# RolandFaure/Hairsplitter

Measured on AMD Instinct MI355X. Metric: aligned read-bp/sec through call_variants+separate_reads, higher is better.
Workload: dtype u8

## Files before the change

### hairsplitter_amd/csrc/hs_kernels_graph.hip

```cpp
#pragma once

namespace hsdev {

static __device__ __forceinline__ float wave_max_f01(float v) { return __int_as_float(wave_max_i32(__float_as_int(v))); }

template <int FILTER>
static __device__ __forceinline__ void next_level(const float* __restrict__ dv, int m, int lane, float cur, float below, float above,
                                                  int extra_zeros, float* v_out, int* c_out) {
    float best = -1.f;
    for (int j = lane; j < m; j += 64) {
        const float d = dv[j];
        const bool ok = FILTER == 0 ? (d != 1.f) : (d > below && d != 1.f && d < above);
        if (ok && d < cur && d > best) best = d;
    }
    if (FILTER == 0 && extra_zeros > 0 && 0.f < cur && best < 0.f) best = 0.f;
    const int key = best < 0.f ? -1 : __float_as_int(best);
    const int kmax = wave_max_i32(key);
    const float vv = kmax < 0 ? -1.f : __int_as_float(kmax);
    int c = 0;
    if (kmax >= 0) {
        for (int j = lane; j < m; j += 64) {
            const float d = dv[j];
            const bool ok = FILTER == 0 ? (d != 1.f) : (d > below && d != 1.f && d < above);
            if (ok && d == vv) c++;
        }
        c = wave_sum_i32(c);
        if (FILTER == 0 && vv == 0.f) c += extra_zeros;
    }
    *v_out = vv; *c_out = c;
}

template <bool LM>
__global__ __launch_bounds__(256) void k_read_graph_rows(
    const int32_t* __restrict__ sim, const int32_t* __restrict__ diff, const int64_t* __restrict__ ctg_out_off,
    const int32_t* __restrict__ ctg_n, const int32_t* __restrict__ win_contig, const int64_t* __restrict__ win_mask_off,
    const int32_t* __restrict__ mask_ids, const int32_t* __restrict__ row_win, const int64_t* __restrict__ win_bits_off,
    int row_base, int n_rows, float below, int cap, unsigned long long* __restrict__ bits, unsigned long long* __restrict__ amb_head ,
    int32_t* __restrict__ amb_rows, int amb_cap, const int64_t* __restrict__ win_mat_off, int es ,
    long long* __restrict__ amb_stage_off , int32_t* __restrict__ stage_sim, int32_t* __restrict__ stage_diff,
    long long stage_cap, const int32_t* __restrict__ pos_rank , const int64_t* __restrict__ rank_off) {
    extern __shared__ unsigned char s_dyn[];
    const int lane = lane_id();
    const int wv = wave_id(), waves = (int)(blockDim.x >> 6);
    const int row = row_base + (int)blockIdx.x * waves + wv;
    if (row >= row_base + n_rows) return;
    float* __restrict__ dv = reinterpret_cast<float*>(s_dyn) + (size_t)wv * 2 * cap;
    int* __restrict__ tv = reinterpret_cast<int*>(dv + cap);
    const int w = row_win[row];
    const int64_t m0 = win_mask_off[w];
    const int m = (int)(win_mask_off[w + 1] - m0);
    const int i = row - (int)m0;
    const int c = win_contig[w];
    const int N = ctg_n[c];
    const int32_t* __restrict__ ids = mask_ids + m0;
    const int r1 = ids[i];
    const int32_t* __restrict__ prk = (!LM && pos_rank) ? pos_rank + rank_off[c] : nullptr;
    const int r1k = prk ? prk[r1] : r1;
    const int32_t* __restrict__ srow = LM ? sim + (win_mat_off[w] + (int64_t)i * m) * es : sim + (ctg_out_off[c] + (int64_t)r1k * N) * es;
    const int32_t* __restrict__ drow = LM ? diff + (win_mat_off[w] + (int64_t)i * m) * es : diff + (ctg_out_off[c] + (int64_t)r1k * N) * es;
    auto give_up = [&]() {
        const int len = LM ? m : N;
        long long so = -1;
        if (lane == 0) {
            const long long k = (long long)atomicAdd(&amb_head[0], 1ull);
            if (k < amb_cap) {
                amb_rows[k] = row;
                if (stage_sim) { so = (long long)atomicAdd(&amb_head[1], (unsigned long long)len); if (so + len > stage_cap) so = -1; }
                amb_stage_off[k] = so;
            }
        }
        so = (long long)(((unsigned long long)(unsigned)__builtin_amdgcn_readlane((int)(so & 0xffffffffll), 0)) |
                         ((unsigned long long)(unsigned)__builtin_amdgcn_readlane((int)((unsigned long long)so >> 32), 0) << 32));
        if (so >= 0) for (int j = lane; j < len; j += 64) { const int64_t at = (int64_t)(prk ? prk[j] : j) * es; stage_sim[so + j] = srow[at]; stage_diff[so + j] = drow[at]; }
    };
    if (m > cap || N < 2 || !(below >= 0.f)) { give_up(); return; }

    int max_compat = 0;
    bool nan_l = false;
    for (int j = lane; j < m; j += 64) {
        const int r = ids[j];
        const int64_t at = (int64_t)(LM ? j : (prk ? prk[r] : r)) * es;
        const int s = srow[at], dd = drow[at];
        float d = 0.f;
        if (LM) {
            if (r != r1) {
                const float df = (float)(dd - 1 > 0 ? dd - 1 : 0);
                d = 1.f - df / (float)(s + dd);
                if (s > max_compat) max_compat = s;
            }
        } else if (r != r1 && s > 0) {
            const float df = (float)(dd - 1 > 0 ? dd - 1 : 0);
            d = 1.f - df / (float)(s + dd);
            if (s > max_compat) max_compat = s;
        }
        dv[j] = d; tv[j] = r != r1 ? s + dd : 0x7fffffff;
    }
    max_compat = wave_max_i32(max_compat);
    const double thr = 0.7 * (double)max_compat;
    for (int j = lane; j < m; j += 64) {
        if ((double)tv[j] < thr) dv[j] = 0.f;
        if (LM && dv[j] != dv[j]) nan_l = true;
    }
    wave_lds_sync();
    if (LM && __ballot(nan_l) != 0ull) { give_up(); return; }

    const int extra_zeros = N - m;
    float s0, s1; int c0, ones = 0;
    {
        float best = 0.f;
        for (int j = lane; j < m; j += 64) { const float d = dv[j]; if (d > best) best = d; if (d == 1.f) ones++; }
        s0 = wave_max_f01(best);
        ones = wave_sum_i32(ones);
        int cnt = 0; float second = -1.f;
        for (int j = lane; j < m; j += 64) { const float d = dv[j]; if (d == s0) cnt++; else if (d > second) second = d; }
        c0 = wave_sum_i32(cnt) + (s0 == 0.f ? extra_zeros : 0);
        if (extra_zeros > 0 && s0 > 0.f && second < 0.f) second = 0.f;
        const int key = second < 0.f ? -1 : __float_as_int(second);
        const int kmax = wave_max_i32(key);
        s1 = c0 >= 2 ? s0 : (kmax < 0 ? -1.f : __int_as_float(kmax));
    }
    float above = s0 - (s0 - s1) * 3;
    if (above == 1.f && ones < N) {
        const int idx = (ones + 4) < (N - 1) ? (ones + 4) : (N - 1);
        int k = idx - ones;
        float cur = 2.f, v = 0.f; int cc = 0;
        for (int it = 0; it < 5; ++it) {
            next_level<0>(dv, m, lane, cur, below, above, extra_zeros, &v, &cc);
            if (cc == 0) { v = 0.f; break; }
            if (k < cc) break;
            k -= cc; cur = v;
        }
        above = v;
    }
    const int mw64 = (m + 63) >> 6;
    unsigned long long* __restrict__ wb = bits + win_bits_off[w];
    int nA = 0;
    for (int j = lane; j < m; j += 64) { const float d = dv[j]; if (d > below && (d == 1.f || d >= above)) nA++; }
    nA = wave_sum_i32(nA);
    float cut = 3.f;
    if (nA < 5) {
        const int need = 5 - nA;
        int nB = 0;
        for (int j = lane; j < m; j += 64) { const float d = dv[j]; if (d > below && d != 1.f && d < above) nB++; }
        nB = wave_sum_i32(nB);
        if (nB > 0 && nB <= need) cut = -1.f;
        else if (nB > need) {
            int remaining = need; float cur = 2.f, v = 0.f; int cc = 0;
            bool ambiguous = false;
            for (int it = 0; it < 5; ++it) {
                next_level<1>(dv, m, lane, cur, below, above, 0, &v, &cc);
                if (remaining <= cc) { ambiguous = remaining != cc; break; }
                remaining -= cc; cur = v;
            }
            if (ambiguous) { give_up(); return; }
            cut = v;
        }
    }
    for (int j = lane; j < m; j += 64) {
        const float d = dv[j];
        const bool take = d > below && ((d == 1.f || d >= above) || (d != 1.f && d < above && d >= cut));
        if (take) {
            atomicOr(&wb[(int64_t)i * mw64 + (j >> 6)], 1ull << (j & 63));
            atomicOr(&wb[(int64_t)j * mw64 + (i >> 6)], 1ull << (i & 63));
        }
    }
}

__global__ __launch_bounds__(256) void k_read_graph_fetch_rows(
    const int32_t* __restrict__ sim, const int32_t* __restrict__ diff, const int64_t* __restrict__ src_off,
    const int32_t* __restrict__ len, const int64_t* __restrict__ dst_off, int32_t* __restrict__ out_sim, int32_t* __restrict__ out_diff, int es) {
    const int k = (int)blockIdx.x;
    const int n = len[k];
    for (int j = (int)threadIdx.x; j < n; j += 256) { out_sim[dst_off[k] + j] = sim[(src_off[k] + j) * es]; out_diff[dst_off[k] + j] = diff[(src_off[k] + j) * es]; }
}

__global__ __launch_bounds__(256) void k_read_graph_patch(const int64_t* __restrict__ base, const int32_t* __restrict__ mw64,
                                                         const int32_t* __restrict__ pi, const int32_t* __restrict__ pj, int n,
                                                         unsigned long long* __restrict__ bits) {
    const int k = (int)(blockIdx.x * 256 + threadIdx.x);
    if (k >= n) return;
    unsigned long long* wb = bits + base[k];
    atomicOr(&wb[(int64_t)pi[k] * mw64[k] + (pj[k] >> 6)], 1ull << (pj[k] & 63));
    atomicOr(&wb[(int64_t)pj[k] * mw64[k] + (pi[k] >> 6)], 1ull << (pi[k] & 63));
}

__global__ __launch_bounds__(256) void k_read_graph_degrees(const unsigned long long* __restrict__ bits, const int32_t* __restrict__ row_win,
                                                           const int64_t* __restrict__ win_mask_off, const int64_t* __restrict__ win_bits_off,
                                                           int n_rows, int32_t* __restrict__ deg) {
    const int row = (int)(blockIdx.x * 256 + threadIdx.x);
    if (row >= n_rows) return;
    const int w = row_win[row];
    const int m = (int)(win_mask_off[w + 1] - win_mask_off[w]);
    const int mw64 = (m + 63) >> 6;
    const unsigned long long* p = bits + win_bits_off[w] + (int64_t)(row - win_mask_off[w]) * mw64;
    int d = 0;
    for (int k = 0; k < mw64; ++k) d += __popcll(p[k]);
    deg[row] = d;
}

#define HS_SCAN_TILE 4096
__global__ __launch_bounds__(256) void k_scan_tile_sums(const int32_t* __restrict__ in, int n, long long* __restrict__ tile_sum) {
    __shared__ int s_w[4];
    const int t = (int)threadIdx.x;
    const int64_t base = (int64_t)blockIdx.x * HS_SCAN_TILE;
    int s = 0;
#pragma unroll
    for (int k = 0; k < HS_SCAN_TILE / 256; ++k) { const int64_t i = base + k * 256 + t; if (i < n) s += in[i]; }
    s = wave_sum_i32(s);
    if ((t & 63) == 0) s_w[t >> 6] = s;
    __syncthreads();
    if (t == 0) tile_sum[blockIdx.x] = (long long)s_w[0] + s_w[1] + s_w[2] + s_w[3];
}

__global__ __launch_bounds__(1024) void k_scan_tile_offsets(const long long* __restrict__ tile_sum, int n_tiles, long long* __restrict__ tile_off,
                                                           int64_t* __restrict__ total_out) {
    __shared__ long long s_part[1024];
    const int t = (int)threadIdx.x;
    long long carry = 0;
    for (int base = 0; base < n_tiles; base += 1024) {
        const long long v = base + t < n_tiles ? tile_sum[base + t] : 0;
        s_part[t] = v;
        __syncthreads();
        for (int d = 1; d < 1024; d <<= 1) {
            const long long a = t >= d ? s_part[t - d] : 0;
            __syncthreads();
            s_part[t] += a;
            __syncthreads();
        }
        if (base + t < n_tiles) tile_off[base + t] = carry + s_part[t] - v;
        carry += s_part[1023];
        __syncthreads();
    }
    if (t == 0) *total_out = carry;
}

__global__ __launch_bounds__(256) void k_scan_apply(const int32_t* __restrict__ in, int n, const long long* __restrict__ tile_off,
                                                    int64_t* __restrict__ out) {
    __shared__ int s_w[2][4];
    const int t = (int)threadIdx.x, lane = t & 63, wv = t >> 6;
    const int64_t base = (int64_t)blockIdx.x * HS_SCAN_TILE;
    long long run = tile_off[blockIdx.x];
#pragma unroll 1
    for (int k = 0; k < HS_SCAN_TILE / 256; ++k) {
        const int64_t i = base + k * 256 + t;
        const int v = i < n ? in[i] : 0;
        const int incl = wave_scan_incl(v);
        if (lane == 63) s_w[k & 1][wv] = incl;
        __syncthreads();
        const int w0 = s_w[k & 1][0], w1 = s_w[k & 1][1], w2 = s_w[k & 1][2], w3 = s_w[k & 1][3];
        const int before = (wv > 0 ? w0 : 0) + (wv > 1 ? w1 : 0) + (wv > 2 ? w2 : 0);
        if (i < n) out[i] = run + before + incl - v;
        run += (long long)w0 + w1 + w2 + w3;
    }
}

__global__ __launch_bounds__(256) void k_read_graph_fill(const unsigned long long* __restrict__ bits, const int32_t* __restrict__ row_win,
                                                        const int64_t* __restrict__ win_mask_off, const int64_t* __restrict__ win_bits_off,
                                                        const int64_t* __restrict__ nbr_off, int n_rows, int32_t* __restrict__ nbr) {
    const int row = (int)(blockIdx.x * 256 + threadIdx.x);
    if (row >= n_rows) return;
    const int w = row_win[row];
    const int64_t m0 = win_mask_off[w];
    const int m = (int)(win_mask_off[w + 1] - m0);
    const int mw64 = (m + 63) >> 6;
    const unsigned long long* p = bits + win_bits_off[w] + (int64_t)(row - m0) * mw64;
    int32_t* o = nbr + nbr_off[row];
    for (int k = 0; k < mw64; ++k) {
        unsigned long long x = p[k];
        while (x) { const int b = __builtin_ctzll(x); x &= x - 1; *o++ = (k << 6) + b; }
    }
}

}
```

### hairsplitter_amd/csrc/hs_sr_backend.inc

```
struct GraphRows {
    DBuf d_oo, d_n, d_wc, d_row0, d_ids, d_rw, d_bo, d_fe, d_rank, d_rank_off, d_pos_rank;
    bool by_pos = false;
    UploadPack pack;
    DBuf d_off, d_nbr, d_visit, d_visit_n, d_prog_info, d_prog_bytes, d_prog_steps, d_prog_adj;
    int64_t rows = 0, rows_dev = 0, total = 0;
    bool total_exact = true;
    int W = 0, max_m = 1;
    std::vector<int32_t> win_m;
    DBuf d_bits, d_amb, d_deg, d_scan, d_wmo, d_ltw, d_lti, d_ltj, d_wsim, d_wdiff, d_stage, d_src, d_len, d_dst, d_os, d_od, d_pb, d_pm, d_pi, d_pj;
    UploadPack pk_amb, pk_patch;
    HBuf h_amb, h_rows, h_deg, h_nbr;
    std::vector<int32_t> row_win;
    std::vector<int64_t> win_bits_off, win_mat_off;
    std::vector<int32_t> lt_w, lt_i, lt_j;
    int Wd = 0, Wmx = 0, rows_mx = 0;
    int row_waves = 0; int64_t n_late = 0;
    size_t amb_cap = 0;
    int64_t stage_cap = 0, stage_hint = 0;
    EventPair ev;
    bool timed = false, begun = false;
    const int32_t* d_sim = nullptr; const int32_t* d_diff = nullptr; int es = 1;
    std::vector<int64_t> ctg_out_off; std::vector<int32_t> ctg_n;
    float* k_ms = nullptr;
};

struct PlaneRows { const uint64_t* d_alt = nullptr; const uint64_t* d_ref = nullptr; const int64_t* d_plane_off = nullptr; const int32_t* d_words = nullptr; };

static int graph_rows_begin(const int32_t* d_sim, const int32_t* d_diff, const std::vector<int64_t>& ctg_out_off, const std::vector<int32_t>& ctg_n_matrix,
                            const hs::SrWindowSet& ws, GraphRows& G, hipStream_t stream, float* k_ms, KernelClock* kc = nullptr,
                            const PlaneRows* planes = nullptr, int es = 1 ) {
    G.ctg_n = ws.ctg_reads.empty() ? ctg_n_matrix : ws.ctg_reads;
    G.ctg_out_off = ctg_out_off;
    const std::vector<int32_t>& ctg_n = G.ctg_n;
    const int W = (int)ws.win_contig.size();
    G.W = W; G.rows = ws.rows(); G.total = 0; G.total_exact = true; G.max_m = 1; G.begun = true; G.timed = false; G.k_ms = k_ms;
    G.d_sim = d_sim; G.d_diff = d_diff; G.es = es; G.row_waves = 0; G.n_late = 0;
    if (G.rows > 0x7fffffff) { set_error("read graphs: too many rows"); return HS_EINVAL; }
    const int rows = (int)G.rows;
    const int Wd = ws.n_dev_windows;
    const int Wmx = ws.ctg_reads.empty() ? Wd : ws.n_matrix_windows;
    const int rows_dev = (int)ws.win_row0[(size_t)Wd];
    const int rows_mx = (int)ws.win_row0[(size_t)Wmx];
    G.rows_dev = rows_dev; G.Wd = Wd; G.Wmx = Wmx; G.rows_mx = rows_mx;
    if (Wmx < Wd && (!planes || !planes->d_alt)) { set_error("read graphs: low-memory windows without bit rows"); return HS_EINVAL; }
    if ((int64_t)ws.host_off.size() != (int64_t)(rows - rows_dev) + 1 && rows != rows_dev) { set_error("read graphs: host rows do not match the window set"); return HS_EINVAL; }
    std::vector<int32_t>& row_win = G.row_win; row_win.assign((size_t)rows_dev, 0);
    std::vector<int64_t>& win_bits_off = G.win_bits_off; win_bits_off.assign((size_t)Wd + 1, 0);
    G.win_m.resize((size_t)W);
    int max_m_dev = 1, max_len = 1;
    for (int w = 0; w < W; ++w) {
        const int64_t m0 = ws.win_row0[(size_t)w], m = ws.win_row0[(size_t)w + 1] - m0;
        G.win_m[(size_t)w] = (int32_t)m;
        G.max_m = std::max(G.max_m, (int)m);
        if (w < Wd) {
            for (int64_t r = 0; r < m; ++r) row_win[(size_t)(m0 + r)] = w;
            win_bits_off[(size_t)w + 1] = win_bits_off[(size_t)w] + m * ((m + 63) >> 6);
            max_m_dev = std::max(max_m_dev, (int)m);
            max_len = std::max(max_len, w < Wmx ? ctg_n[(size_t)ws.win_contig[(size_t)w]] : (int)m);
        }
    }
    std::vector<int64_t>& win_mat_off = G.win_mat_off; win_mat_off.assign((size_t)Wd + 1, 0);
    std::vector<int32_t>& lt_w = G.lt_w; std::vector<int32_t>& lt_i = G.lt_i; std::vector<int32_t>& lt_j = G.lt_j;
    lt_w.clear(); lt_i.clear(); lt_j.clear();
    for (int w = 0; w < Wd; ++w) {
        const int64_t m = w >= Wmx ? G.win_m[(size_t)w] : 0;
        win_mat_off[(size_t)w + 1] = win_mat_off[(size_t)w] + m * m;
        const int nt = (int)((m + 63) / 64);
        for (int i = 0; i < nt; ++i) for (int j = 0; j < nt; ++j) { lt_w.push_back(w); lt_i.push_back(i); lt_j.push_back(j); }
    }
    if (Wmx < Wd) { G.pack.add(win_mat_off, G.d_wmo); G.pack.add(lt_w, G.d_ltw); G.pack.add(lt_i, G.d_lti); G.pack.add(lt_j, G.d_ltj); }
    G.pack.add(ctg_out_off, G.d_oo);
    G.pack.add(ctg_n, G.d_n);
    G.pack.add(ws.win_contig, G.d_wc);
    G.pack.add(ws.win_row0, G.d_row0);
    G.pack.add(ws.mask_ids, G.d_ids);
    G.pack.add(row_win, G.d_rw);
    G.pack.add(win_bits_off, G.d_bo);
    G.pack.add(ws.win_final_empty, G.d_fe);
    G.pack.add(ws.rank, G.d_rank);
    G.pack.add(ws.ctg_rank_off, G.d_rank_off);
    G.by_pos = !ws.pos_rank.empty();
    if (G.by_pos) G.pack.add(ws.pos_rank, G.d_pos_rank);
    if (int rc = G.pack.commit(stream)) return rc;
    if (int rc = G.d_off.alloc(((size_t)rows + 1) * 8 + 32)) return rc;
    if (int rc = G.d_visit.alloc(std::max<size_t>((size_t)rows, 1) * 4)) return rc;
    if (int rc = G.d_visit_n.alloc(std::max<size_t>((size_t)W, 1) * 4)) return rc;
    if (rows == 0) { hipLaunchKernelGGL(hsdev::k_fill16, dim3(1), dim3(64), 0, stream, G.d_off.as<uint4>(), 1ll, 0u); HS_HIP(hipGetLastError()); return HS_OK; }
    if (int rc = G.d_deg.alloc((size_t)rows * 4)) return rc;
    if (int rc = G.ev.init()) return rc;
    if (rows_dev > 0) {
        if (rows_mx > 0 && !d_sim) { set_error("read graphs before simdiff"); return HS_EINVAL; }
        const size_t bits_bytes = ((size_t)win_bits_off.back() * 8 + 15) & ~(size_t)15;
        if (int rc = G.d_bits.alloc(std::max<size_t>(bits_bytes, 16))) return rc;
        G.amb_cap = (size_t)rows_dev;
        G.stage_cap = std::max<int64_t>(G.stage_hint + G.stage_hint / 2, 64 * (int64_t)max_len);
        const size_t amb_bytes = 16 + (((size_t)G.amb_cap * 4 + 15) & ~(size_t)15) + (((size_t)G.amb_cap * 8 + 15) & ~(size_t)15);
        if (int rc = G.d_amb.alloc(amb_bytes)) return rc;
        if (int rc = G.d_stage.alloc((size_t)G.stage_cap * 8 + 32)) return rc;
        hipLaunchKernelGGL(hsdev::k_fill16, dim3((unsigned)std::min<size_t>(256, bits_bytes / 4096 + 1)), dim3(256), 0, stream, G.d_bits.as<uint4>(), (long long)(std::max<size_t>(bits_bytes, 16) / 16), 0u);
        hipLaunchKernelGGL(hsdev::k_fill16, dim3(1), dim3(64), 0, stream, G.d_amb.as<uint4>(), 1ll, 0u);
        unsigned long long* amb_head = G.d_amb.as<unsigned long long>();
        int32_t* amb_rows = reinterpret_cast<int32_t*>((char*)G.d_amb.p + 16);
        long long* amb_so = reinterpret_cast<long long*>((char*)G.d_amb.p + 16 + (((size_t)G.amb_cap * 4 + 15) & ~(size_t)15));
        int32_t* st_sim = G.d_stage.as<int32_t>(); int32_t* st_diff = st_sim + (((size_t)G.stage_cap + 3) & ~(size_t)3);
        int cap = ((max_m_dev + 63) / 64) * 64, waves = 4;
        if ((size_t)cap * 8 * 4 > 57344) waves = 1;
        if ((size_t)cap * 8 > 57344) cap = 7168;
        const float below = 1 - ws.error_rate * 2;
        G.row_waves = waves;
        HS_HIP(ev_rec(G.ev.a, stream));
        if (rows_mx > 0) {
            if (kc) { if (int rc = kc->begin(HS_K_GRAPH_ROWS, stream)) return rc; }
            hipLaunchKernelGGL(hsdev::k_read_graph_rows<false>, dim3((rows_mx + waves - 1) / waves), dim3(64 * waves), (size_t)cap * 8 * waves, stream, d_sim, d_diff,
                               G.d_oo.as<int64_t>(), G.d_n.as<int32_t>(), G.d_wc.as<int32_t>(), G.d_row0.as<int64_t>(), G.d_ids.as<int32_t>(), G.d_rw.as<int32_t>(),
                               G.d_bo.as<int64_t>(), 0, rows_mx, below, cap, G.d_bits.as<unsigned long long>(), amb_head, amb_rows, (int)G.amb_cap,
                               (const int64_t*)nullptr, es, amb_so, st_sim, st_diff, (long long)G.stage_cap, G.by_pos ? G.d_pos_rank.as<int32_t>() : nullptr, G.d_rank_off.as<int64_t>());
            HS_HIP(hipGetLastError());
            if (kc) {
                int64_t by = 0;
                for (int w = 0; w < Wmx; ++w) { const int64_t m = G.win_m[(size_t)w]; by += m * (8 * m + (m + 7) / 8); }
                if (int rc = kc->end(by, stream)) return rc;
            }
        }
        if (rows_dev > rows_mx) {
            const size_t mat = (size_t)win_mat_off.back();
            if (int rc = G.d_wsim.alloc(std::max<size_t>(mat, 1) * 8)) return rc;
            G.d_wdiff.release(); G.d_wdiff.p = (char*)G.d_wsim.p + 4; G.d_wdiff.bytes = 0; G.d_wdiff.cap = 0; G.d_wdiff.view = true;
            if (kc) { if (int rc = kc->begin(HS_K_SIMDIFF, stream)) return rc; }
            hipLaunchKernelGGL(hsdev::k_simdiff_windows, dim3((unsigned)lt_w.size()), dim3(256), 0, stream, planes->d_alt, planes->d_ref, planes->d_plane_off, planes->d_words,
                               G.d_wc.as<int32_t>(), G.d_row0.as<int64_t>(), G.d_ids.as<int32_t>(), G.d_wmo.as<int64_t>(), G.d_ltw.as<int32_t>(), G.d_lti.as<int32_t>(),
                               G.d_ltj.as<int32_t>(), G.d_wsim.as<int32_t>(), G.d_wdiff.as<int32_t>(), 2);
            HS_HIP(hipGetLastError());
            if (kc) { if (int rc = kc->end(8 * (int64_t)mat, stream)) return rc; }
            if (kc) { if (int rc = kc->begin(HS_K_GRAPH_ROWS, stream)) return rc; }
            const int n_lm = rows_dev - rows_mx;
            hipLaunchKernelGGL(hsdev::k_read_graph_rows<true>, dim3((n_lm + waves - 1) / waves), dim3(64 * waves), (size_t)cap * 8 * waves, stream, G.d_wsim.as<int32_t>(),
                               G.d_wdiff.as<int32_t>(), G.d_oo.as<int64_t>(), G.d_n.as<int32_t>(), G.d_wc.as<int32_t>(), G.d_row0.as<int64_t>(), G.d_ids.as<int32_t>(),
                               G.d_rw.as<int32_t>(), G.d_bo.as<int64_t>(), rows_mx, n_lm, below, cap, G.d_bits.as<unsigned long long>(), amb_head, amb_rows, (int)G.amb_cap,
                               G.d_wmo.as<int64_t>(), 2, amb_so, st_sim, st_diff, (long long)G.stage_cap, (const int32_t*)nullptr, (const int64_t*)nullptr);
            HS_HIP(hipGetLastError());
            if (kc) { if (int rc = kc->end(8 * (int64_t)mat, stream)) return rc; }
        }
        HS_HIP(ev_rec(G.ev.b, stream));
        G.timed = true;
        const size_t rows_part = ((size_t)G.amb_cap * 4 + 15) & ~(size_t)15, stage_half = (((size_t)G.stage_cap + 3) & ~(size_t)3) * 4;
        if (int rc = G.h_amb.alloc(amb_bytes + 2 * stage_half + 64)) return rc;
        Shipment sh;
        char* hb = (char*)G.h_amb.p;
        sh.add(hb, G.d_amb.p, 16);
        sh.add_counted(hb + 16, (char*)G.d_amb.p + 16, reinterpret_cast<const long long*>(amb_head), 4, (long long)G.amb_cap);
        sh.add_counted(hb + 16 + rows_part, (char*)G.d_amb.p + 16 + rows_part, reinterpret_cast<const long long*>(amb_head), 8, (long long)G.amb_cap);
        sh.add_counted(hb + amb_bytes, st_sim, reinterpret_cast<const long long*>(amb_head + 1), 4, G.stage_cap);
        sh.add_counted(hb + amb_bytes + stage_half, st_diff, reinterpret_cast<const long long*>(amb_head + 1), 4, G.stage_cap);
        if (kc) { if (int rc = kc->begin(HS_K_SHIP, stream)) return rc; }
        if (int rc = sh.launch(stream, 16)) return rc;
        if (kc) { if (int rc = kc->end(0, stream)) return rc; }
    }
    return HS_OK;
}

static int graph_rows_end(const hs::SrWindowSet& ws, GraphRows& G, hipStream_t stream, int64_t* rows_on_host, KernelClock* kc = nullptr) {
    if (rows_on_host) *rows_on_host = 0;
    const int rows = (int)G.rows, rows_dev = (int)G.rows_dev, rows_mx = G.rows_mx, Wd = G.Wd, Wmx = G.Wmx, W = G.W;
    if (rows == 0) return HS_OK;
    const std::vector<int32_t>& ctg_n = G.ctg_n;
    const std::vector<int32_t>& row_win = G.row_win;
    const std::vector<int64_t>& win_bits_off = G.win_bits_off;
    const std::vector<int64_t>& win_mat_off = G.win_mat_off;
    if (rows_dev > 0) {
        if (int rc = stream_wait(stream)) return rc;
        const size_t rows_part = ((size_t)G.amb_cap * 4 + 15) & ~(size_t)15, amb_bytes = 16 + rows_part + (((size_t)G.amb_cap * 8 + 15) & ~(size_t)15), stage_half = (((size_t)G.stage_cap + 3) & ~(size_t)3) * 4;
        const char* hb = (const char*)G.h_amb.p;
        const int64_t n_amb = (int64_t)((const unsigned long long*)hb)[0];
        const int64_t staged = (int64_t)((const unsigned long long*)hb)[1];
        G.stage_hint = staged;
        if (n_amb > (int64_t)G.amb_cap) { set_error("read graphs: more undecided rows than rows"); return HS_EINVAL; }
        if (n_amb > 0) {
            const int32_t* amb_rows = (const int32_t*)(hb + 16);
            const long long* amb_so = (const long long*)(hb + 16 + rows_part);
            const int32_t* st_sim = (const int32_t*)(hb + amb_bytes); const int32_t* st_diff = (const int32_t*)(hb + amb_bytes + stage_half);
            std::vector<int32_t> order((size_t)n_amb);
            for (int64_t k = 0; k < n_amb; ++k) order[(size_t)k] = (int32_t)k;
            std::sort(order.begin(), order.end(), [&](int32_t x, int32_t y) { return amb_rows[x] < amb_rows[y]; });
            std::vector<int32_t> late;
            for (int32_t k : order) if (amb_so[k] < 0) late.push_back(k);
            G.n_late = (int64_t)late.size();
            std::vector<int64_t> late_dst((size_t)late.size() + 1, 0);
            const int32_t* late_sim = nullptr; const int32_t* late_diff = nullptr;
            if (!late.empty()) {
                std::vector<int64_t> src(late.size()); std::vector<int32_t> len(late.size());
                int n_mx = 0;
                for (size_t q = 0; q < late.size(); ++q) {
                    const int row = amb_rows[late[q]];
                    const int w = row_win[(size_t)row];
                    const int c = ws.win_contig[(size_t)w];
                    const int N = ctg_n[(size_t)c];
                    const int r1 = ws.mask_ids[(size_t)row];
                    if (row < rows_mx) { const int r1k = G.by_pos ? ws.pos_rank[(size_t)ws.ctg_rank_off[(size_t)c] + (size_t)r1] : r1; src[q] = G.ctg_out_off[(size_t)c] + (int64_t)r1k * N; len[q] = N; n_mx++; }
                    else { const int64_t m = G.win_m[(size_t)w]; src[q] = win_mat_off[(size_t)w] + (int64_t)(row - ws.win_row0[(size_t)w]) * m; len[q] = (int32_t)m; }
                    late_dst[q + 1] = late_dst[q] + len[q];
                }
                G.pk_amb.add(src, G.d_src); G.pk_amb.add(len, G.d_len); G.pk_amb.add(late_dst, G.d_dst);
                if (int rc = G.pk_amb.commit(stream)) return rc;
                if (int rc = G.d_os.alloc((size_t)late_dst.back() * 4 + 16)) return rc;
                if (int rc = G.d_od.alloc((size_t)late_dst.back() * 4 + 16)) return rc;
                if (n_mx > 0)
                    hipLaunchKernelGGL(hsdev::k_read_graph_fetch_rows, dim3(n_mx), dim3(256), 0, stream, G.d_sim, G.d_diff, G.d_src.as<int64_t>(), G.d_len.as<int32_t>(),
                                       G.d_dst.as<int64_t>(), G.d_os.as<int32_t>(), G.d_od.as<int32_t>(), G.es);
                if ((int)late.size() > n_mx)
                    hipLaunchKernelGGL(hsdev::k_read_graph_fetch_rows, dim3((unsigned)late.size() - n_mx), dim3(256), 0, stream, G.d_wsim.as<int32_t>(), G.d_wdiff.as<int32_t>(),
                                       G.d_src.as<int64_t>() + n_mx, G.d_len.as<int32_t>() + n_mx, G.d_dst.as<int64_t>() + n_mx, G.d_os.as<int32_t>(), G.d_od.as<int32_t>(), 2);
                HS_HIP(hipGetLastError());
                const size_t row_bytes = (((size_t)late_dst.back() * 4) + 15) & ~(size_t)15;
                if (int rc = G.h_rows.alloc(2 * row_bytes + 16)) return rc;
                Shipment sh; sh.add(G.h_rows.p, G.d_os.p, row_bytes); sh.add((char*)G.h_rows.p + row_bytes, G.d_od.p, row_bytes);
                if (int rc = sh.launch(stream, 16)) return rc;
                if (int rc_w = stream_wait(stream)) return rc_w;
                late_sim = (const int32_t*)G.h_rows.p; late_diff = (const int32_t*)((const char*)G.h_rows.p + row_bytes);
                G.stage_hint = std::max<int64_t>(G.stage_hint, staged + late_dst.back());
            }
            std::vector<int64_t> pbase; std::vector<int32_t> pmw, pi, pj;
            std::vector<uint8_t> mask;
            std::vector<int> picked;
            size_t late_q = 0;
            for (int32_t k : order) {
                const int row = amb_rows[k];
                const int w = row_win[(size_t)row];
                const int64_t m0 = ws.win_row0[(size_t)w];
                const int m = (int)(ws.win_row0[(size_t)w + 1] - m0);
                const int32_t* ids = ws.mask_ids.data() + m0;
                const int N = ctg_n[(size_t)ws.win_contig[(size_t)w]];
                const int32_t* rs; const int32_t* rd;
                std::vector<int32_t> perm_s, perm_d;
                if (late_q < late.size() && late[late_q] == k) {
                    rs = late_sim + late_dst[late_q]; rd = late_diff + late_dst[late_q]; late_q++;
                    if (G.by_pos && row < rows_mx) {
                        const int32_t* pr = ws.pos_rank.data() + ws.ctg_rank_off[(size_t)ws.win_contig[(size_t)w]];
                        perm_s.resize((size_t)N); perm_d.resize((size_t)N);
                        for (int r = 0; r < N; ++r) { perm_s[(size_t)r] = rs[pr[r]]; perm_d[(size_t)r] = rd[pr[r]]; }
                        rs = perm_s.data(); rd = perm_d.data();
                    }
                }
                else { rs = st_sim + amb_so[k]; rd = st_diff + amb_so[k]; }
                mask.assign((size_t)N, 0);
                for (int j = 0; j < m; ++j) mask[(size_t)ids[j]] = 1;
                if (row < rows_mx) hs::sr_pick_row_sorted(rs, rd, N, ids[row - m0], mask.data(), ws.error_rate, picked);
                else hs::sr_pick_row_sorted_low_memory(rs, rd, ids, m, (int)(row - m0), N, mask.data(), ws.error_rate, picked);
                for (int nb : picked) {
                    const int j = (int)(std::lower_bound(ids, ids + m, nb) - ids);
                    pbase.push_back(win_bits_off[(size_t)w]); pmw.push_back((m + 63) >> 6); pi.push_back((int32_t)(row - m0)); pj.push_back(j);
                }
            }
            if (!pi.empty()) {
                G.pk_patch.add(pbase, G.d_pb); G.pk_patch.add(pmw, G.d_pm); G.pk_patch.add(pi, G.d_pi); G.pk_patch.add(pj, G.d_pj);
                if (int rc = G.pk_patch.commit(stream)) return rc;
                const int np = (int)pi.size();
                hipLaunchKernelGGL(hsdev::k_read_graph_patch, dim3((np + 255) / 256), dim3(256), 0, stream, G.d_pb.as<int64_t>(), G.d_pm.as<int32_t>(), G.d_pi.as<int32_t>(),
                                   G.d_pj.as<int32_t>(), np, G.d_bits.as<unsigned long long>());
                HS_HIP(hipGetLastError());
            }
            if (rows_on_host) *rows_on_host = n_amb;
            if (std::getenv("HS_TIMING") && Wmx < Wd) {
                int64_t n_lm = 0; for (int64_t k = 0; k < n_amb; ++k) n_lm += amb_rows[k] >= rows_mx;
                std::fprintf(stderr, "[hs timing] sr: low-memory path on the device: %d windows, %d rows, %ld of them resolved on the host (NaN distances / std::sort ties)\n",
                             Wd - Wmx, rows_dev - rows_mx, (long)n_lm);
            }
        } else if (std::getenv("HS_TIMING") && Wmx < Wd)
            std::fprintf(stderr, "[hs timing] sr: low-memory path on the device: %d windows, %d rows, none resolved on the host\n", Wd - Wmx, rows_dev - rows_mx);
        if (kc) { if (int rc = kc->begin(HS_K_GRAPH_CSR, stream)) return rc; }
        hipLaunchKernelGGL(hsdev::k_read_graph_degrees, dim3((rows_dev + 255) / 256), dim3(256), 0, stream, G.d_bits.as<unsigned long long>(), G.d_rw.as<int32_t>(),
                           G.d_row0.as<int64_t>(), G.d_bo.as<int64_t>(), rows_dev, G.d_deg.as<int32_t>());
        HS_HIP(hipGetLastError());
        if (kc) { if (int rc = kc->end((int64_t)win_bits_off.back() * 8 + 4 * (int64_t)rows_dev, stream)) return rc; }
    }
    if (rows > rows_dev) {
        const size_t nh = (size_t)(rows - rows_dev);
        if (int rc = G.h_deg.alloc(nh * 4 + 16)) return rc;
        int32_t* hd = (int32_t*)G.h_deg.p;
        for (size_t r = 0; r < nh; ++r) hd[r] = (int32_t)(ws.host_off[r + 1] - ws.host_off[r]);
        HS_HIP(HS_COPY_ASYNC(G.d_deg.as<int32_t>() + rows_dev, hd, nh * 4, hipMemcpyHostToDevice, stream));
    }
    if (int rc = exclusive_scan_launch(G.d_deg.as<int32_t>(), rows, G.d_off.as<int64_t>(), G.d_scan, stream)) return rc;
    int64_t bound = (int64_t)ws.host_nbr.size();
    for (int w = 0; w < Wd; ++w) bound += (int64_t)G.win_m[(size_t)w] * G.win_m[(size_t)w];
    int64_t total = bound;
    G.total_exact = false;
    if (!ws.host_nbr.empty() || bound > ((int64_t)1 << 28)) {
        if (int rc = d2h_pinned(&total, G.d_off.as<int64_t>() + rows, 8, stream)) return rc;
        G.total_exact = true;
    }
    G.total = total;
    if (int rc = G.d_nbr.alloc(std::max<size_t>((size_t)total, 1) * 4)) return rc;
    if (total > 0) {
        if (rows_dev > 0) {
            if (kc) { if (int rc = kc->begin(HS_K_GRAPH_CSR, stream)) return rc; }
            hipLaunchKernelGGL(hsdev::k_read_graph_fill, dim3((rows_dev + 255) / 256), dim3(256), 0, stream, G.d_bits.as<unsigned long long>(), G.d_rw.as<int32_t>(),
                               G.d_row0.as<int64_t>(), G.d_bo.as<int64_t>(), G.d_off.as<int64_t>(), rows_dev, G.d_nbr.as<int32_t>());
            HS_HIP(hipGetLastError());
            if (kc) { if (int rc = kc->end((int64_t)win_bits_off.back() * 8 + 4 * (G.total_exact ? total : (int64_t)rows_dev * 20), stream)) return rc; }
        }
        if (!ws.host_nbr.empty()) {
            const size_t nb = ws.host_nbr.size() * 4;
            if (int rc = G.h_nbr.alloc(nb)) return rc;
            std::memcpy(G.h_nbr.p, ws.host_nbr.data(), nb);
            HS_HIP(HS_COPY_ASYNC(G.d_nbr.as<int32_t>() + (total - (int64_t)ws.host_nbr.size()), G.h_nbr.p, nb, hipMemcpyHostToDevice, stream));
        }
    }
    {
        const int cap = std::min(((G.max_m + 63) / 64) * 64, 8192);
        if (int rc = G.d_prog_info.alloc(std::max<size_t>((size_t)rows, 1) * 4)) return rc;
        if (int rc = G.d_prog_bytes.alloc((size_t)total + 15 * (size_t)rows + 64)) return rc;
        const size_t steps_bytes = (std::max<size_t>((size_t)W, 1) * 4 + 15) & ~(size_t)15;
        if (int rc = G.d_prog_steps.alloc(steps_bytes)) return rc;
        if (int rc = G.d_prog_adj.alloc(std::max<size_t>((size_t)rows, 1) * 8)) return rc;
        hipLaunchKernelGGL(hsdev::k_fill16, dim3((unsigned)std::min<size_t>(64, steps_bytes / 4096 + 1)), dim3(256), 0, stream, G.d_prog_steps.as<uint4>(), (long long)(steps_bytes / 16), 0u);
        if (kc) { if (int rc = kc->begin(HS_K_VISIT_LISTS, stream)) return rc; }
        hipLaunchKernelGGL(hsdev::k_cw_visit_lists, dim3((unsigned)W), dim3(256), (size_t)cap * 4, stream, G.d_off.as<int64_t>(), G.d_nbr.as<int32_t>(), G.d_row0.as<int64_t>(),
                           G.d_ids.as<int32_t>(), G.d_wc.as<int32_t>(), G.d_rank_off.as<int64_t>(), G.d_rank.as<int32_t>(), W, cap, G.d_visit.as<int32_t>(),
                           G.d_visit_n.as<int32_t>(), G.d_prog_info.as<uint32_t>(), G.d_prog_bytes.as<uint8_t>(), G.d_prog_steps.as<int32_t>(),
                           G.d_prog_adj.as<unsigned long long>());
        HS_HIP(hipGetLastError());
        if (kc) { if (int rc = kc->end(20 * (int64_t)rows, stream)) return rc; }
    }
    return HS_OK;
}
static int graph_rows_settle(GraphRows& G, KernelClock* kc) {
    if (kc) kc->flush();
    if (G.timed) { G.timed = false; float m = 0; if (int rc = G.ev.ms(&m)) return rc; if (G.k_ms) *G.k_ms += m; }
    return HS_OK;
}
static int graph_rows_build(const int32_t* d_sim, const int32_t* d_diff, const std::vector<int64_t>& ctg_out_off, const std::vector<int32_t>& ctg_n_matrix,
                            const hs::SrWindowSet& ws, GraphRows& G, hipStream_t stream, int64_t* rows_on_host, float* k_ms, KernelClock* kc = nullptr,
                            const PlaneRows* planes = nullptr, int es = 1) {
    if (int rc = graph_rows_begin(d_sim, d_diff, ctg_out_off, ctg_n_matrix, ws, G, stream, k_ms, kc, planes, es)) return rc;
    if (int rc = graph_rows_end(ws, G, stream, rows_on_host, kc)) return rc;
    if (G.rows > 0 && !G.total_exact) { int64_t t = 0; if (int rc = d2h_pinned(&t, G.d_off.as<int64_t>() + G.rows, 8, stream)) return rc; G.total = t; G.total_exact = true; }
    else if (int rc_w = stream_wait(stream)) return rc_w;
    return graph_rows_settle(G, kc);
}

struct HipSrOps : hs::SrDeviceOps {
    hipStream_t stream = nullptr;
    DBuf d_sim, d_diff;
    std::vector<int64_t> sd_out_off;
    std::vector<int32_t> sd_n;
    GraphRows G;
    KernelClock kc;

    struct SimdiffInFlight {
        DBuf d_alt, d_ref, d_sr, d_sa, d_sc, d_cb, d_po, d_n, d_pn, d_w, d_oo, t_c, t_i, t_j, d_bc, d_bw, d_rb, d_orig, d_rng;
        std::vector<int32_t> tc, ti, tj, blk_c, blk_w;
        UploadPack pk;
        EventPair ev;
        float* k_ms = nullptr;
    };
    std::unique_ptr<SimdiffInFlight> sd_flight;
    int settle_simdiff(bool account = true) {
        if (!sd_flight) return HS_OK;
        float m = 0;
        int rc = (sd_flight->ev.a || k5_waited) ? HS_OK : stream_wait_quiet(stream);
        if (!rc) rc = sd_flight->ev.ms(&m);
        if (!rc && account && sd_flight->k_ms) *sd_flight->k_ms += m;
        sd_flight.reset();
        return rc;
    }
    bool k5_waited = false;
    ~HipSrOps() override { (void)settle_simdiff(false); }

    DBuf d_col_off, d_col_idx, d_col_code;
    UploadPack col_pack;
    const hs::CwChain* resident_cols = nullptr;
    bool adopted = false;
    int64_t adopted_cols = 0, adopted_entries = 0;
    DBuf cols_block;
    void adopt_columns(HipCvOps& cv) {
        std::swap(cols_block, cv.d_pk);
        char* base = (char*)cols_block.p;
        auto view = [&](DBuf& d, size_t off, size_t bytes) { d.release(); d.p = base + off; d.bytes = bytes; d.cap = 0; d.view = true; };
        view(d_col_off, cv.pk_layout.off, ((size_t)cv.snp_count + 1) * 8);
        view(d_col_idx, cv.pk_layout.idx, (size_t)cv.snp_entries * 4);
        view(d_col_code, cv.pk_layout.code, (size_t)cv.snp_entries);
        adopted = true; adopted_cols = cv.snp_count; adopted_entries = cv.snp_entries;
    }
    bool columns_resident() const override { return adopted; }
    bool low_memory_graphs() const override { static const bool host = std::getenv("HS_LOW_MEMORY_GRAPHS_ON_HOST") != nullptr; return !host; }
    void drop_resident_columns() override { adopted = false; resident_cols = nullptr; }
    int fetch_columns(std::vector<int32_t>& idx, std::vector<uint8_t>& code) override {
        if (!adopted) { set_error("fetch_columns: no resident columns"); return HS_EINVAL; }
        idx.resize((size_t)adopted_entries); code.resize((size_t)adopted_entries);
        if (adopted_entries == 0) return HS_OK;
        if (int rc = d2h_pinned(idx.data(), d_col_idx.p, (size_t)adopted_entries * 4, stream)) return rc;
        return d2h_pinned(code.data(), d_col_code.p, (size_t)adopted_entries, stream);
    }
    int window_masks(const std::vector<int64_t>& col_a, const std::vector<int64_t>& col_b, const std::vector<int64_t>& slot_off,
                     std::vector<int32_t>& ids, std::vector<int32_t>& win_m) override {
        if (!adopted) { set_error("window_masks: no resident columns"); return HS_EINVAL; }
        const int W = (int)col_a.size();
        const int64_t total = slot_off.back();
        ids.resize((size_t)total); win_m.assign((size_t)W, 0);
        if (W == 0) return HS_OK;
        DBuf d_a, d_b, d_so, d_ids;
        UploadPack pk;
        pk.add(col_a, d_a); pk.add(col_b, d_b); pk.add(slot_off, d_so);
        if (int rc = pk.commit(stream)) return rc;
        const size_t ids_bytes = ((size_t)total * 4 + 255) & ~(size_t)255;
        if (int rc = d_ids.alloc(ids_bytes + (size_t)W * 4 + 16)) return rc;
        int32_t* const dm = reinterpret_cast<int32_t*>((char*)d_ids.p + ids_bytes);
        if (int rc = kc.begin(HS_K_WINDOW_MASKS, stream)) return rc;
        hipLaunchKernelGGL(hsdev::k_window_masks, dim3((unsigned)((W + 3) / 4)), dim3(256), 0, stream, d_col_off.as<int64_t>(), d_col_idx.as<int32_t>(), d_a.as<int64_t>(),
                           d_b.as<int64_t>(), d_so.as<int64_t>(), W, d_ids.as<int32_t>(), dm);
        HS_HIP(hipGetLastError());
        if (int rc = kc.end(8 * total + 4 * (int64_t)W, stream)) return rc;
        HBuf h_ids;
        if (int rc = h_ids.alloc(ids_bytes + (size_t)W * 4 + 16)) return rc;
        { Shipment sh; sh.add(h_ids.p, d_ids.p, ids_bytes + (size_t)W * 4); if (int rc = sh.launch(stream, 32)) return rc; }
        if (int rc = stream_wait(stream)) return rc;
        k5_waited = true;
        if (total) std::memcpy(ids.data(), h_ids.p, (size_t)total * 4);
        std::memcpy(win_m.data(), (const char*)h_ids.p + ids_bytes, (size_t)W * 4);
        kc.flush();
        return HS_OK;
    }
    int simdiff_columns(const hs::SimdiffJob& job, float* k_ms) override {
// ... 408 lines not shown
```

Baseline: 130.0 billion.

## Process graph rows per window with register-resident rows and shared-memory bitmaps

Replaces the per-row graph kernel for matrix-backed windows with a per-window kernel. For windows of up to 64 reads, each row lives in registers (one lane per column), the next row's sim/diff values are prefetched, and adjacency bits are built in shared memory before one store to global. This removes LDS traffic, per-bit global atomics and the separate full zero-fill of the bitmap, which is now zeroed only for the later windows. The logic is factored into a generic row rule over LDS or register backends, which adds template complexity. XCD-aware window striding is also added.

New measurement: 112.2 billion. 0.863x the previous value.

```diff
diff --git a/hairsplitter_amd/csrc/hs_kernels_graph.hip b/hairsplitter_amd/csrc/hs_kernels_graph.hip
--- a/hairsplitter_amd/csrc/hs_kernels_graph.hip
+++ b/hairsplitter_amd/csrc/hs_kernels_graph.hip
@@ -4,30 +4,168 @@
 
 static __device__ __forceinline__ float wave_max_f01(float v) { return __int_as_float(wave_max_i32(__float_as_int(v))); }
 
-template <int FILTER>
-static __device__ __forceinline__ void next_level(const float* __restrict__ dv, int m, int lane, float cur, float below, float above,
-                                                  int extra_zeros, float* v_out, int* c_out) {
+template <int FILTER, class Row>
+static __device__ __forceinline__ void next_level(Row& R, float cur, float below, float above, int extra_zeros, float* v_out, int* c_out) {
     float best = -1.f;
-    for (int j = lane; j < m; j += 64) {
-        const float d = dv[j];
+    R.each([&](int, float& d, int&) {
         const bool ok = FILTER == 0 ? (d != 1.f) : (d > below && d != 1.f && d < above);
         if (ok && d < cur && d > best) best = d;
-    }
+    });
     if (FILTER == 0 && extra_zeros > 0 && 0.f < cur && best < 0.f) best = 0.f;
     const int key = best < 0.f ? -1 : __float_as_int(best);
     const int kmax = wave_max_i32(key);
     const float vv = kmax < 0 ? -1.f : __int_as_float(kmax);
     int c = 0;
     if (kmax >= 0) {
-        for (int j = lane; j < m; j += 64) {
-            const float d = dv[j];
+        R.each([&](int, float& d, int&) {
             const bool ok = FILTER == 0 ? (d != 1.f) : (d > below && d != 1.f && d < above);
             if (ok && d == vv) c++;
-        }
-        c = wave_sum_i32(c);
+        });
+        c = R.count(c);
         if (FILTER == 0 && vv == 0.f) c += extra_zeros;
     }
     *v_out = vv; *c_out = c;
+}
+
+struct RowLds {
+    float* __restrict__ dv; int* __restrict__ tv; int m, lane;
+    template <class F> __device__ __forceinline__ void each(F&& f) { for (int j = lane; j < m; j += 64) f(j, dv[j], tv[j]); }
+    __device__ __forceinline__ int count(int c) const { return wave_sum_i32(c); }
+};
+struct RowRegs {
+    float d; int t; int m, lane;
+    template <class F> __device__ __forceinline__ void each(F&& f) { if (lane < m) f(lane, d, t); }
+    __device__ __forceinline__ int count(int c) const { return __popcll(__ballot(c != 0)); }
+};
+
+template <bool LM, class Row, class Entry, class Link>
+static __device__ __forceinline__ bool graph_row_rule(Row& R, int r1, int N, float below, Entry&& entry, Link&& link) {
+    int max_compat = 0;
+    bool nan_l = false;
+    R.each([&](int j, float& dj, int& tj) {
+        int r, s, dd;
+        entry(j, &r, &s, &dd);
+        float d = 0.f;
+        if (LM) {
+            if (r != r1) {
+                const float df = (float)(dd - 1 > 0 ? dd - 1 : 0);
+                d = 1.f - df / (float)(s + dd);
+                if (s > max_compat) max_compat = s;
+            }
+        } else if (r != r1 && s > 0) {
+            const float df = (float)(dd - 1 > 0 ? dd - 1 : 0);
+            d = 1.f - df / (float)(s + dd);
+            if (s > max_compat) max_compat = s;
+        }
+        dj = d; tj = r != r1 ? s + dd : 0x7fffffff;
+    });
+    max_compat = wave_max_i32(max_compat);
+    const double thr = 0.7 * (double)max_compat;
+    R.each([&](int, float& dj, int& tj) {
+        if ((double)tj < thr) dj = 0.f;
+        if (LM && dj != dj) nan_l = true;
+    });
+    if (LM && __ballot(nan_l) != 0ull) return false;
+
+    const int extra_zeros = N - R.m;
+    float s0, s1; int c0, ones = 0;
+    {
+        float best = 0.f;
+        R.each([&](int, float& d, int&) { if (d > best) best = d; if (d == 1.f) ones++; });
+        s0 = wave_max_f01(best);
+        ones = R.count(ones);
+        int cnt = 0; float second = -1.f;
+        R.each([&](int, float& d, int&) { if (d == s0) cnt++; else if (d > second) second = d; });
+        c0 = R.count(cnt) + (s0 == 0.f ? extra_zeros : 0);
+        if (extra_zeros > 0 && s0 > 0.f && second < 0.f) second = 0.f;
+        const int key = second < 0.f ? -1 : __float_as_int(second);
+        const int kmax = wave_max_i32(key);
+        s1 = c0 >= 2 ? s0 : (kmax < 0 ? -1.f : __int_as_float(kmax));
+    }
+    float above = s0 - (s0 - s1) * 3;
+    if (above == 1.f && ones < N) {
+        const int idx = (ones + 4) < (N - 1) ? (ones + 4) : (N - 1);
+        int k = idx - ones;
+        float cur = 2.f, v = 0.f; int cc = 0;
+        for (int it = 0; it < 5; ++it) {
+            next_level<0>(R, cur, below, above, extra_zeros, &v, &cc);
+            if (cc == 0) { v = 0.f; break; }
+            if (k < cc) break;
+            k -= cc; cur = v;
+        }
+        above = v;
+    }
+    int nA = 0;
+    R.each([&](int, float& d, int&) { if (d > below && (d == 1.f || d >= above)) nA++; });
+    nA = R.count(nA);
+    float cut = 3.f;
+    if (nA < 5) {
+        const int need = 5 - nA;
+        int nB = 0;
+        R.each([&](int, float& d, int&) { if (d > below && d != 1.f && d < above) nB++; });
+        nB = R.count(nB);
+        if (nB > 0 && nB <= need) cut = -1.f;
+        else if (nB > need) {
+            int remaining = need; float cur = 2.f, v = 0.f; int cc = 0;
+            bool ambiguous = false;
+            for (int it = 0; it < 5; ++it) {
+                next_level<1>(R, cur, below, above, 0, &v, &cc);
+                if (remaining <= cc) { ambiguous = remaining != cc; break; }
+                remaining -= cc; cur = v;
+            }
+            if (ambiguous) return false;
+            cut = v;
+        }
+    }
+    R.each([&](int j, float& d, int&) {
+        const bool take = d > below && ((d == 1.f || d >= above) || (d != 1.f && d < above && d >= cut));
+        if (take) link(j);
+    });
+    return true;
+}
+
+struct GraphAmb {
+    unsigned long long* __restrict__ head;
+    int32_t* __restrict__ rows; int cap;
+    long long* __restrict__ stage_off;
+    int32_t* __restrict__ stage_sim; int32_t* __restrict__ stage_diff; long long stage_cap;
+};
+
+static __device__ __forceinline__ void graph_row_give_up(const GraphAmb& A, int row, int len, const int32_t* __restrict__ srow, const int32_t* __restrict__ drow,
+                                                         const int32_t* __restrict__ prk, int es, int lane) {
+    long long so = -1;
+    if (lane == 0) {
+        const long long k = (long long)atomicAdd(&A.head[0], 1ull);
+        if (k < A.cap) {
+            A.rows[k] = row;
+            if (A.stage_sim) { so = (long long)atomicAdd(&A.head[1], (unsigned long long)len); if (so + len > A.stage_cap) so = -1; }
+            A.stage_off[k] = so;
+        }
+    }
+    so = (long long)(((unsigned long long)(unsigned)__builtin_amdgcn_readlane((int)(so & 0xffffffffll), 0)) |
+                     ((unsigned long long)(unsigned)__builtin_amdgcn_readlane((int)((unsigned long long)so >> 32), 0) << 32));
+    if (so >= 0) for (int j = lane; j < len; j += 64) { const int64_t at = (int64_t)(prk ? prk[j] : j) * es; A.stage_sim[so + j] = srow[at]; A.stage_diff[so + j] = drow[at]; }
+}
+
+template <bool LM>
+static __device__ __forceinline__ void graph_row_general(const GraphAmb& A, const int32_t* __restrict__ srow, const int32_t* __restrict__ drow, const int32_t* __restrict__ ids,
+                                                         const int32_t* __restrict__ prk, int es, int row, int i, int m, int N, float below, int cap,
+                                                         float* __restrict__ dv, int* __restrict__ tv, unsigned long long* __restrict__ wb) {
+    const int lane = lane_id();
+    if (m > cap || N < 2 || !(below >= 0.f)) { graph_row_give_up(A, row, LM ? m : N, srow, drow, prk, es, lane); return; }
+    const int mw64 = (m + 63) >> 6;
+    RowLds R{dv, tv, m, lane};
+    const bool decided = graph_row_rule<LM>(R, ids[i], N, below,
+        [&](int j, int* r, int* s, int* dd) {
+            *r = ids[j];
+            const int64_t at = (int64_t)(LM ? j : (prk ? prk[*r] : *r)) * es;
+            *s = srow[at]; *dd = drow[at];
+        },
+        [&](int j) {
+            atomicOr(&wb[(int64_t)i * mw64 + (j >> 6)], 1ull << (j & 63));
+            atomicOr(&wb[(int64_t)j * mw64 + (i >> 6)], 1ull << (i & 63));
+        });
+    if (!decided) graph_row_give_up(A, row, LM ? m : N, srow, drow, prk, es, lane);
 }
 
 template <bool LM>
@@ -40,7 +178,6 @@
     long long* __restrict__ amb_stage_off , int32_t* __restrict__ stage_sim, int32_t* __restrict__ stage_diff,
     long long stage_cap, const int32_t* __restrict__ pos_rank , const int64_t* __restrict__ rank_off) {
     extern __shared__ unsigned char s_dyn[];
-    const int lane = lane_id();
     const int wv = wave_id(), waves = (int)(blockDim.x >> 6);
     const int row = row_base + (int)blockIdx.x * waves + wv;
     if (row >= row_base + n_rows) return;
@@ -58,112 +195,74 @@
     const int r1k = prk ? prk[r1] : r1;
     const int32_t* __restrict__ srow = LM ? sim + (win_mat_off[w] + (int64_t)i * m) * es : sim + (ctg_out_off[c] + (int64_t)r1k * N) * es;
     const int32_t* __restrict__ drow = LM ? diff + (win_mat_off[w] + (int64_t)i * m) * es : diff + (ctg_out_off[c] + (int64_t)r1k * N) * es;
-    auto give_up = [&]() {
-        const int len = LM ? m : N;
-        long long so = -1;
-        if (lane == 0) {
-            const long long k = (long long)atomicAdd(&amb_head[0], 1ull);
-            if (k < amb_cap) {
-                amb_rows[k] = row;
-                if (stage_sim) { so = (long long)atomicAdd(&amb_head[1], (unsigned long long)len); if (so + len > stage_cap) so = -1; }
-                amb_stage_off[k] = so;
-            }
-        }
-        so = (long long)(((unsigned long long)(unsigned)__builtin_amdgcn_readlane((int)(so & 0xffffffffll), 0)) |
-                         ((unsigned long long)(unsigned)__builtin_amdgcn_readlane((int)((unsigned long long)so >> 32), 0) << 32));
-        if (so >= 0) for (int j = lane; j < len; j += 64) { const int64_t at = (int64_t)(prk ? prk[j] : j) * es; stage_sim[so + j] = srow[at]; stage_diff[so + j] = drow[at]; }
-    };
-    if (m > cap || N < 2 || !(below >= 0.f)) { give_up(); return; }
-
-    int max_compat = 0;
-    bool nan_l = false;
-    for (int j = lane; j < m; j += 64) {
-        const int r = ids[j];
-        const int64_t at = (int64_t)(LM ? j : (prk ? prk[r] : r)) * es;
-        const int s = srow[at], dd = drow[at];
-        float d = 0.f;
-        if (LM) {
-            if (r != r1) {
-                const float df = (float)(dd - 1 > 0 ? dd - 1 : 0);
-                d = 1.f - df / (float)(s + dd);
-                if (s > max_compat) max_compat = s;
-            }
-        } else if (r != r1 && s > 0) {
-            const float df = (float)(dd - 1 > 0 ? dd - 1 : 0);
-            d = 1.f - df / (float)(s + dd);
-            if (s > max_compat) max_compat = s;
-        }
-        dv[j] = d; tv[j] = r != r1 ? s + dd : 0x7fffffff;
-    }
-    max_compat = wave_max_i32(max_compat);
-    const double thr = 0.7 * (double)max_compat;
-    for (int j = lane; j < m; j += 64) {
-        if ((double)tv[j] < thr) dv[j] = 0.f;
-        if (LM && dv[j] != dv[j]) nan_l = true;
-    }
-    wave_lds_sync();
-    if (LM && __ballot(nan_l) != 0ull) { give_up(); return; }
-
-    const int extra_zeros = N - m;
-    float s0, s1; int c0, ones = 0;
-    {
-        float best = 0.f;
-        for (int j = lane; j < m; j += 64) { const float d = dv[j]; if (d > best) best = d; if (d == 1.f) ones++; }
-        s0 = wave_max_f01(best);
-        ones = wave_sum_i32(ones);
-        int cnt = 0; float second = -1.f;
-        for (int j = lane; j < m; j += 64) { const float d = dv[j]; if (d == s0) cnt++; else if (d > second) second = d; }
-        c0 = wave_sum_i32(cnt) + (s0 == 0.f ? extra_zeros : 0);
-        if (extra_zeros > 0 && s0 > 0.f && second < 0.f) second = 0.f;
-        const int key = second < 0.f ? -1 : __float_as_int(second);
-        const int kmax = wave_max_i32(key);
-        s1 = c0 >= 2 ? s0 : (kmax < 0 ? -1.f : __int_as_float(kmax));
-    }
-    float above = s0 - (s0 - s1) * 3;
-    if (above == 1.f && ones < N) {
-        const int idx = (ones + 4) < (N - 1) ? (ones + 4) : (N - 1);
-        int k = idx - ones;
-        float cur = 2.f, v = 0.f; int cc = 0;
-        for (int it = 0; it < 5; ++it) {
-            next_level<0>(dv, m, lane, cur, below, above, extra_zeros, &v, &cc);
-            if (cc == 0) { v = 0.f; break; }
-            if (k < cc) break;
-            k -= cc; cur = v;
-        }
-        above = v;
-    }
-    const int mw64 = (m + 63) >> 6;
+    const GraphAmb A{amb_head, amb_rows, amb_cap, amb_stage_off, stage_sim, stage_diff, stage_cap};
+    graph_row_general<LM>(A, srow, drow, ids, prk, es, row, i, m, N, below, cap, dv, tv, bits + win_bits_off[w]);
+}
+
+__global__ __launch_bounds__(256) void k_read_graph_rows_window(
+    const int32_t* __restrict__ sim, const int32_t* __restrict__ diff, const int64_t* __restrict__ ctg_out_off,
+    const int32_t* __restrict__ ctg_n, const int32_t* __restrict__ win_contig, const int64_t* __restrict__ win_mask_off,
+    const int32_t* __restrict__ mask_ids, const int64_t* __restrict__ win_bits_off, int n_win, float below, int cap ,
+    unsigned long long* __restrict__ bits, unsigned long long* __restrict__ amb_head, int32_t* __restrict__ amb_rows, int amb_cap, int es,
+    long long* __restrict__ amb_stage_off, int32_t* __restrict__ stage_sim, int32_t* __restrict__ stage_diff, long long stage_cap,
+    const int32_t* __restrict__ pos_rank, const int64_t* __restrict__ rank_off) {
+    extern __shared__ unsigned char s_dyn[];
+    __shared__ unsigned long long s_bits[64];
+    const int t = (int)threadIdx.x, lane = lane_id();
+    const int wv = wave_id(), waves = (int)(blockDim.x >> 6);
+    const int per_xcd = (n_win + 7) >> 3;
+    const int w = (int)(blockIdx.x & 7u) * per_xcd + (int)(blockIdx.x >> 3);
+    if (w >= n_win) return;
+    const int64_t m0 = win_mask_off[w];
+    const int m = (int)(win_mask_off[w + 1] - m0);
+    if (m == 0) return;
+    const int c = win_contig[w];
+    const int N = ctg_n[c];
+    const int32_t* __restrict__ ids = mask_ids + m0;
+    const int32_t* __restrict__ prk = pos_rank ? pos_rank + rank_off[c] : nullptr;
+    const int64_t mat = ctg_out_off[c];
     unsigned long long* __restrict__ wb = bits + win_bits_off[w];
-    int nA = 0;
-    for (int j = lane; j < m; j += 64) { const float d = dv[j]; if (d > below && (d == 1.f || d >= above)) nA++; }
-    nA = wave_sum_i32(nA);
-    float cut = 3.f;
-    if (nA < 5) {
-        const int need = 5 - nA;
-        int nB = 0;
-        for (int j = lane; j < m; j += 64) { const float d = dv[j]; if (d > below && d != 1.f && d < above) nB++; }
-        nB = wave_sum_i32(nB);
-        if (nB > 0 && nB <= need) cut = -1.f;
-        else if (nB > need) {
-            int remaining = need; float cur = 2.f, v = 0.f; int cc = 0;
-            bool ambiguous = false;
-            for (int it = 0; it < 5; ++it) {
-                next_level<1>(dv, m, lane, cur, below, above, 0, &v, &cc);
-                if (remaining <= cc) { ambiguous = remaining != cc; break; }
-                remaining -= cc; cur = v;
-            }
-            if (ambiguous) { give_up(); return; }
-            cut = v;
-        }
-    }
-    for (int j = lane; j < m; j += 64) {
-        const float d = dv[j];
-        const bool take = d > below && ((d == 1.f || d >= above) || (d != 1.f && d < above && d >= cut));
-        if (take) {
-            atomicOr(&wb[(int64_t)i * mw64 + (j >> 6)], 1ull << (j & 63));
-            atomicOr(&wb[(int64_t)j * mw64 + (i >> 6)], 1ull << (i & 63));
-        }
-    }
+    const GraphAmb A{amb_head, amb_rows, amb_cap, amb_stage_off, stage_sim, stage_diff, stage_cap};
+    if (m > 64) {
+        const int64_t words = (int64_t)m * ((m + 63) >> 6);
+        for (int64_t k = t; k < words; k += blockDim.x) wb[k] = 0ull;
+        __threadfence();
+        __syncthreads();
+        float* __restrict__ dv = reinterpret_cast<float*>(s_dyn) + (size_t)wv * 2 * cap;
+        int* __restrict__ tv = reinterpret_cast<int*>(dv + cap);
+        for (int i = wv; i < m; i += waves) {
+            const int r1 = ids[i];
+            const int64_t at = (mat + (int64_t)(prk ? prk[r1] : r1) * N) * es;
+            graph_row_general<false>(A, sim + at, diff + at, ids, prk, es, (int)m0 + i, i, m, N, below, cap, dv, tv, wb);
+        }
+        return;
+    }
+    if (t < 64) s_bits[t] = 0ull;
+    __syncthreads();
+    const bool to_host = N < 2 || !(below >= 0.f);
+    const int id = lane < m ? ids[lane] : 0;
+    const int64_t col = (int64_t)((lane < m && prk) ? prk[id] : id);
+    auto row_at = [&](int i) { return (mat + (int64_t)__builtin_amdgcn_readlane((int)col, i) * N) * es; };
+    int s_next = 0, dd_next = 0;
+    if (wv < m && lane < m && !to_host) { const int64_t at = row_at(wv) + col * es; s_next = sim[at]; dd_next = diff[at]; }
+    for (int i = wv; i < m; i += waves) {
+        const int64_t at_i = row_at(i);
+        const int s = s_next, dd = dd_next;
+        if (i + waves < m && lane < m && !to_host) { const int64_t at = row_at(i + waves) + col * es; s_next = sim[at]; dd_next = diff[at]; }
+        bool taken = false;
+        bool decided = !to_host;
+        if (decided) {
+            RowRegs R{0.f, 0, m, lane};
+            decided = graph_row_rule<false>(R, __builtin_amdgcn_readlane(id, i), N, below,
+                                            [&](int, int* r, int* ps, int* pdd) { *r = id; *ps = s; *pdd = dd; }, [&](int) { taken = true; });
+        }
+        if (!decided) { graph_row_give_up(A, (int)m0 + i, N, sim + at_i, diff + at_i, prk, es, lane); continue; }
+        const unsigned long long linked = __ballot(taken);
+        if (lane == 0 && linked) atomicOr(&s_bits[i], linked);
+        if (taken) atomicOr(&s_bits[lane], 1ull << i);
+    }
+    __syncthreads();
+    if (t < m) wb[t] = s_bits[t];
 }
 
 __global__ __launch_bounds__(256) void k_read_graph_fetch_rows(
diff --git a/hairsplitter_amd/csrc/hs_sr_backend.inc b/hairsplitter_amd/csrc/hs_sr_backend.inc
--- a/hairsplitter_amd/csrc/hs_sr_backend.inc
+++ b/hairsplitter_amd/csrc/hs_sr_backend.inc
@@ -97,7 +97,12 @@
         const size_t amb_bytes = 16 + (((size_t)G.amb_cap * 4 + 15) & ~(size_t)15) + (((size_t)G.amb_cap * 8 + 15) & ~(size_t)15);
         if (int rc = G.d_amb.alloc(amb_bytes)) return rc;
         if (int rc = G.d_stage.alloc((size_t)G.stage_cap * 8 + 32)) return rc;
-        hipLaunchKernelGGL(hsdev::k_fill16, dim3((unsigned)std::min<size_t>(256, bits_bytes / 4096 + 1)), dim3(256), 0, stream, G.d_bits.as<uint4>(), (long long)(std::max<size_t>(bits_bytes, 16) / 16), 0u);
+        if (Wmx < Wd) {
+            const size_t lm_from = ((size_t)win_bits_off[(size_t)Wmx] * 8) & ~(size_t)15, lm_bytes = bits_bytes - lm_from;
+            if (lm_bytes > 0)
+                hipLaunchKernelGGL(hsdev::k_fill16, dim3((unsigned)std::min<size_t>(256, lm_bytes / 4096 + 1)), dim3(256), 0, stream,
+                                   reinterpret_cast<uint4*>((char*)G.d_bits.p + lm_from), (long long)(lm_bytes / 16), 0u);
+        }
         hipLaunchKernelGGL(hsdev::k_fill16, dim3(1), dim3(64), 0, stream, G.d_amb.as<uint4>(), 1ll, 0u);
         unsigned long long* amb_head = G.d_amb.as<unsigned long long>();
         int32_t* amb_rows = reinterpret_cast<int32_t*>((char*)G.d_amb.p + 16);
@@ -111,14 +116,16 @@
         HS_HIP(ev_rec(G.ev.a, stream));
         if (rows_mx > 0) {
             if (kc) { if (int rc = kc->begin(HS_K_GRAPH_ROWS, stream)) return rc; }
-            hipLaunchKernelGGL(hsdev::k_read_graph_rows<false>, dim3((rows_mx + waves - 1) / waves), dim3(64 * waves), (size_t)cap * 8 * waves, stream, d_sim, d_diff,
-                               G.d_oo.as<int64_t>(), G.d_n.as<int32_t>(), G.d_wc.as<int32_t>(), G.d_row0.as<int64_t>(), G.d_ids.as<int32_t>(), G.d_rw.as<int32_t>(),
-                               G.d_bo.as<int64_t>(), 0, rows_mx, below, cap, G.d_bits.as<unsigned long long>(), amb_head, amb_rows, (int)G.amb_cap,
-                               (const int64_t*)nullptr, es, amb_so, st_sim, st_diff, (long long)G.stage_cap, G.by_pos ? G.d_pos_rank.as<int32_t>() : nullptr, G.d_rank_off.as<int64_t>());
+            int max_m_mx = 0;
+            for (int w = 0; w < Wmx; ++w) max_m_mx = std::max(max_m_mx, (int)G.win_m[(size_t)w]);
+            hipLaunchKernelGGL(hsdev::k_read_graph_rows_window, dim3(8u * (((unsigned)Wmx + 7u) / 8u)), dim3(64 * waves), max_m_mx > 64 ? (size_t)cap * 8 * waves : (size_t)0, stream, d_sim, d_diff,
+                               G.d_oo.as<int64_t>(), G.d_n.as<int32_t>(), G.d_wc.as<int32_t>(), G.d_row0.as<int64_t>(), G.d_ids.as<int32_t>(),
+                               G.d_bo.as<int64_t>(), Wmx, below, cap, G.d_bits.as<unsigned long long>(), amb_head, amb_rows, (int)G.amb_cap,
+                               es, amb_so, st_sim, st_diff, (long long)G.stage_cap, G.by_pos ? G.d_pos_rank.as<int32_t>() : nullptr, G.d_rank_off.as<int64_t>());
             HS_HIP(hipGetLastError());
             if (kc) {
                 int64_t by = 0;
-                for (int w = 0; w < Wmx; ++w) { const int64_t m = G.win_m[(size_t)w]; by += m * (8 * m + (m + 7) / 8); }
+                for (int w = 0; w < Wmx; ++w) { const int64_t m = G.win_m[(size_t)w]; by += m * (8 * m + (G.by_pos ? 8 : 4) + 8 * ((m + 63) / 64)); }
                 if (int rc = kc->end(by, stream)) return rc;
             }
         }
```
